# xmindflow/cenet

Hardware: AMD Instinct MI355X
Metric: training images/sec (224x224, 4-class) (higher is better)
Workload: dtype bf16

## Files before the change

cenet_amd/csrc/pvt_mlp.hip:

```cpp
#include "gemm_ring.h"

struct PvtMlpArgs {
  const bf16_t* x;
  const float* ln_g;
  const float* ln_b;
  const bf16_t* w1;
  const float* b1;
  const float* wd;
  const float* bd;
  const bf16_t* w2;
  const float* b2;
  const float* bscale;
  bf16_t* y;
  bf16_t* xn_out;
  float* mean_out;
  float* rstd_out;
  bf16_t* h_out;
  bf16_t* a_out;
  int H, W, HD, tiles_x, tiles_per_img;
  float eps;
};

#ifdef CENET_HOSTSIM_BUILD
#define PVT_WAVE_ID(tid) ((tid) >> 6)
#else
#define PVT_WAVE_ID(tid) __builtin_amdgcn_readfirstlane((tid) >> 6)
#endif

__device__ __forceinline__ float pvt_rcp(float x) {
#ifdef CENET_HOSTSIM_BUILD
  return 1.f / x;
#else
  return __builtin_amdgcn_rcpf(x);
#endif
}
__device__ __forceinline__ float pvt_gelu(float u) { return gelu_as(u); }
template <int LPT>
__device__ __forceinline__ float pvt_subrow_sum(float v) {
#pragma unroll
  for (int o = LPT / 2; o > 0; o >>= 1) v += __shfl_xor(v, o);
  return v;
}

__device__ __forceinline__ void pvt_load_kf64(const bf16_t* src, long ld, unsigned char* img, int wave, int lane) {
  const int S = wave * 64 + lane, row = S >> 3, c = (S & 7) ^ kf_key(row);
  ring_glds16(src + (long)row * ld + 8 * c, img + wave * 1024, lane);
}

template <int BX>
__device__ __forceinline__ void pvt_load_rf(const bf16_t* src, long ld, unsigned char* img, int wave, int lane) {
  constexpr int CH = BX / 8;
#pragma unroll
  for (int j = 0; j < BX / 64; ++j) {
    const int S = (j * 8 + wave) * 64 + lane;
    const int k = S / CH, c = (S % CH) ^ rf_key<BX>(k);
    ring_glds16(src + (long)k * ld + 8 * c, img + (j * 8 + wave) * 1024, lane);
  }
}

template <int C, int PW, int PT, int PTP, int TH, int TW>
__device__ __forceinline__ void pvt_ln_tile(const bf16_t* ximg, const float* ln_g, const float* ln_b, float eps, int H, int W,
                                            int y0, int x0, int halo, unsigned char* XN, bf16_t* xn_out, float* mean_out,
                                            float* rstd_out, int tid) {
  constexpr int LPT = C / 8, TPP = 512 / LPT;
  const int j = tid % LPT, tsub = tid / LPT;
  float gm[8], bt[8];
  {
    const f4 g0 = ld4(ln_g + 8 * j), g1 = ld4(ln_g + 8 * j + 4), b0 = ld4(ln_b + 8 * j), b1 = ld4(ln_b + 8 * j + 4);
#pragma unroll
    for (int e = 0; e < 4; ++e) gm[e] = g0.v[e], gm[4 + e] = g1.v[e], bt[e] = b0.v[e], bt[4 + e] = b1.v[e];
  }
  const float invC = 1.f / C;
#pragma unroll
  for (int p0 = 0; p0 < PTP; p0 += TPP) {
    const int p = p0 + tsub;
    const int ty = p / PW, tx = p - ty * PW;
    const int iy = y0 - halo + ty, ix = x0 - halo + tx;
    const bool ok = p < PT && iy >= 0 && iy < H && ix >= 0 && ix < W;
    float v[8];
    if (ok) ldv<8>(v, ximg + ((long)iy * W + ix) * C + 8 * j);
    else {
#pragma unroll
      for (int e = 0; e < 8; ++e) v[e] = 0.f;
    }
    float s = ((v[0] + v[1]) + (v[2] + v[3])) + ((v[4] + v[5]) + (v[6] + v[7]));
    const float mu = pvt_subrow_sum<LPT>(s) * invC;
    float q = 0.f;
#pragma unroll
    for (int e = 0; e < 8; ++e) {
      const float d = v[e] - mu;
      q += d * d;
    }
    const float rs = rsqrtf(pvt_subrow_sum<LPT>(q) * invC + eps);
    unsigned o[4];
#pragma unroll
    for (int h = 0; h < 4; ++h) {
      const float a0 = ok ? (v[2 * h] - mu) * rs * gm[2 * h] + bt[2 * h] : 0.f;
      const float a1 = ok ? (v[2 * h + 1] - mu) * rs * gm[2 * h + 1] + bt[2 * h + 1] : 0.f;
      o[h] = cenet_pack_bf2(a0, a1);
    }
    if (p < PTP) *(uint4*)(XN + (j >> 3) * (PTP * 128) + p * 128 + ((j & 7) ^ kf_key(p)) * 16) = uint4{o[0], o[1], o[2], o[3]};
    if (xn_out && ok && ty >= halo && ty < halo + TH && tx >= halo && tx < halo + TW) {
      const long tk = (long)iy * W + ix;
      *(uint4*)(xn_out + tk * C + 8 * j) = uint4{o[0], o[1], o[2], o[3]};
      if (j == 0) mean_out[tk] = mu, rstd_out[tk] = rs;
    }
  }
}

template <int C, int TH, int TW>
struct PvtFwdGeo {
  static constexpr int PW = TW + 2, PH = TH + 2, PT = PH * PW, PTP = (PT + 15) / 16 * 16, MTH = PTP / 16;
  static constexpr int NT = TH * TW, MTI = (NT + 15) / 16, SL = TW / 2;
  static constexpr int KB = C / 64, HS = 136;
  static constexpr int XN_B = KB * PTP * 128, A_B = MTI * 16 * 128, W1_B = KB * 8192, W2_B = C * 128, H_B = PTP * HS;
  static constexpr int O_XN = 0, O_A = XN_B, O_W1 = O_A + A_B, O_W2 = O_W1 + W1_B, O_H = O_W2 + W2_B, LDS = O_H + H_B;
};

template <int C, int TH, int TW>
__global__ __launch_bounds__(512, 2) void pvt_mlp_fwd_kernel(PvtMlpArgs a) {
  typedef PvtFwdGeo<C, TH, TW> G;
  constexpr int PW = G::PW, PT = G::PT, PTP = G::PTP, MTH = G::MTH, NT = G::NT, MTI = G::MTI, SL = G::SL, KB = G::KB, HS = G::HS;
  static_assert(C == 64 || C == 128, "channels");
  static_assert(MTI <= 8 && 2 * TH <= 16 && TW % 2 == 0, "tile shape");
  __shared__ __attribute__((aligned(1024))) unsigned char lds[G::LDS];
  unsigned char* const XN = lds + G::O_XN;
  unsigned char* const AI = lds + G::O_A;
  unsigned char* const W1I = lds + G::O_W1;
  unsigned char* const W2I = lds + G::O_W2;
  unsigned char* const HI = lds + G::O_H;

  const int tid = threadIdx.x, lane = tid & 63;
  const int wave = PVT_WAVE_ID(tid);
  const cenet_bid bid = cenet_xcd_block();
  const int b = bid.x / a.tiles_per_img, t = bid.x - b * a.tiles_per_img;
  const int y0 = (t / a.tiles_x) * TH, x0 = (t % a.tiles_x) * TW;
  const long img = (long)b * a.H * a.W;
  const bf16_t* ximg = a.x + img * C;
  const int nslab = a.HD / 64;

#pragma unroll
  for (int kb = 0; kb < KB; ++kb) pvt_load_kf64(a.w1 + kb * 64, C, W1I + kb * 8192, wave, lane);
#pragma unroll
  for (int r = 0; r < C / 64; ++r) pvt_load_kf64(a.w2 + (long)(r * 64) * a.HD, a.HD, W2I + r * 8192, wave, lane);

  pvt_ln_tile<C, PW, PT, PTP, TH, TW>(ximg, a.ln_g, a.ln_b, a.eps, a.H, a.W, y0, x0, 1, XN, a.xn_out ? a.xn_out + img * C : nullptr,
                                      a.mean_out + img, a.rstd_out + img, tid);

  f32x4 acc[C / 16];
#pragma unroll
  for (int i = 0; i < C / 16; ++i) acc[i] = f32x4{0.f, 0.f, 0.f, 0.f};

  const float sc_b = a.bscale ? a.bscale[b] : 1.f;
  const int cp = tid & 31, strip = tid >> 5;
  const int oy = strip >> 1, ox0 = (strip & 1) * SL;
  const bool p2_on = strip < 2 * TH;
  const int ct = wave & 3;

  ring_wait_vm<0>();
  __syncthreads();

  for (int s = 0; s < nslab; ++s) {
    float wdv[18], bdv[2], b1v[4];
    {
      const float* wp = a.wd + (long)(s * 64 + 2 * cp) * 9;
#pragma unroll
      for (int i = 0; i < 9; ++i) {
        const float2 v = *(const float2*)(wp + 2 * i);
        wdv[2 * i] = v.x, wdv[2 * i + 1] = v.y;
      }
      bdv[0] = a.bd[s * 64 + 2 * cp], bdv[1] = a.bd[s * 64 + 2 * cp + 1];
      const f4 bb = ld4(a.b1 + s * 64 + ct * 16 + (lane >> 4) * 4);
      b1v[0] = bb.v[0], b1v[1] = bb.v[1], b1v[2] = bb.v[2], b1v[3] = bb.v[3];
    }
    {
      bf16x8 wf[KB * 2];
#pragma unroll
      for (int k = 0; k < KB * 2; ++k) wf[k] = ring_frag_kf(W1I + (k >> 1) * 8192, ct * 16, k & 1, lane);
      for (int tt = wave >> 2; tt < MTH; tt += 2) {
        f32x4 h = f32x4{0.f, 0.f, 0.f, 0.f};
#pragma unroll
        for (int k = 0; k < KB * 2; ++k) {
          const bf16x8 xf = ring_frag_kf(XN + (k >> 1) * (PTP * 128), tt * 16, k & 1, lane);
          h = __builtin_amdgcn_mfma_f32_16x16x32_bf16(wf[k], xf, h, 0, 0, 0);
        }
        const int p = tt * 16 + (lane & 15);
        const int ty = p / PW, tx = p - ty * PW;
        const int iy = y0 - 1 + ty, ix = x0 - 1 + tx;
        const bool ok = p < PT && iy >= 0 && iy < a.H && ix >= 0 && ix < a.W;
        unsigned o[2];
        o[0] = ok ? cenet_pack_bf2(h[0] + b1v[0], h[1] + b1v[1]) : 0u;
        o[1] = ok ? cenet_pack_bf2(h[2] + b1v[2], h[3] + b1v[3]) : 0u;
        *(uint2*)(HI + p * HS + (ct * 16 + (lane >> 4) * 4) * 2) = uint2{o[0], o[1]};
      }
    }
    __syncthreads();
    if (s + 1 < nslab) {
#pragma unroll
      for (int kb = 0; kb < KB; ++kb) pvt_load_kf64(a.w1 + (long)(s + 1) * 64 * C + kb * 64, C, W1I + kb * 8192, wave, lane);
    }
    unsigned hkeep[SL], akeep[SL];
    if (p2_on) {
      float u[SL][2];
#pragma unroll
      for (int i = 0; i < SL; ++i) u[i][0] = bdv[0], u[i][1] = bdv[1];
      const unsigned char* hp = HI + (oy * PW + ox0) * HS + cp * 4;
#pragma unroll
      for (int kxx = 0; kxx < SL + 2; ++kxx) {
        float h0[3], h1[3];
#pragma unroll
        for (int ky = 0; ky < 3; ++ky) {
          const unsigned v = *(const unsigned*)(hp + (ky * PW + kxx) * HS);
          h0[ky] = __uint_as_float(v << 16);
          h1[ky] = __uint_as_float(v & 0xFFFF0000u);
          if (ky == 1 && kxx >= 1 && kxx <= SL) hkeep[kxx - 1] = v;
        }
#pragma unroll
        for (int kx = 0; kx < 3; ++kx) {
          const int i = kxx - kx;
          if (i >= 0 && i < SL) {
#pragma unroll
            for (int ky = 0; ky < 3; ++ky) {
              u[i][0] += wdv[ky * 3 + kx] * h0[ky];
              u[i][1] += wdv[9 + ky * 3 + kx] * h1[ky];
            }
          }
        }
      }
#pragma unroll
      for (int i = 0; i < SL; ++i) {
        const int row = oy * TW + ox0 + i;
        const float a0 = pvt_gelu(u[i][0]), a1 = pvt_gelu(u[i][1]);
        const unsigned v = cenet_pack_bf2(a0, a1);
        *(unsigned*)(AI + row * 128 + (((cp >> 2) ^ kf_key(row)) * 16) + (cp & 3) * 4) = v;
        akeep[i] = a.bscale ? cenet_pack_bf2(a0 * sc_b, a1 * sc_b) : v;
      }
    }
    ring_wait_vm<0>();
    __syncthreads();
    if (a.h_out && p2_on) {
      const long o = (img + (long)(y0 + oy) * a.W + x0 + ox0) * a.HD + s * 64 + 2 * cp;
#pragma unroll
      for (int i = 0; i < SL; ++i) {
        *(unsigned*)(a.h_out + o + (long)i * a.HD) = hkeep[i];
        *(unsigned*)(a.a_out + o + (long)i * a.HD) = akeep[i];
      }
    }
    if (wave < MTI) {
#pragma unroll
      for (int kc = 0; kc < 2; ++kc) {
        const bf16x8 af = ring_frag_kf(AI, wave * 16, kc, lane);
#pragma unroll
        for (int nt = 0; nt < C / 16; ++nt) {
          const bf16x8 wf = ring_frag_kf(W2I + (nt >> 2) * 8192, (nt & 3) * 16, kc, lane);
          acc[nt] = __builtin_amdgcn_mfma_f32_16x16x32_bf16(wf, af, acc[nt], 0, 0, 0);
        }
      }
    }
    __syncthreads();
    if (s + 1 < nslab) {
#pragma unroll
      for (int r = 0; r < C / 64; ++r)
        pvt_load_kf64(a.w2 + (long)(r * 64) * a.HD + (s + 1) * 64, a.HD, W2I + r * 8192, wave, lane);
    }
  }
  if (wave < MTI) {
    const int ti = wave * 16 + (lane & 15);
    const int ry = ti / TW, rx = ti - ry * TW;
    const int gy = y0 + ry, gx = x0 + rx;
    if (ti < NT && gy < a.H && gx < a.W) {
      const float sc = sc_b;
      const long tok = img + (long)gy * a.W + gx;
#pragma unroll
      for (int nt = 0; nt < C / 16; ++nt) {
        const int n0 = nt * 16 + (lane >> 4) * 4;
        const f4 xr = ld4(a.x + tok * C + n0);
        const f4 bb = ld4(a.b2 + n0);
        f4 o;
#pragma unroll
        for (int e = 0; e < 4; ++e) o.v[e] = xr.v[e] + sc * (acc[nt][e] + bb.v[e]);
        st4(a.y + tok * C + n0, o);
      }
    }
  }
}

__device__ __forceinline__ float pvt_gelu_grad(float u) { return gelu_as_grad(u); }

struct PvtBwdArgs {
  const bf16_t* g;
  const float* bscale;
  const bf16_t* w1;
  const bf16_t* w2;
  const float* wd;
  const float* bd;
  const bf16_t* h;
  bf16_t* gu;
  bf16_t* dh;
  float* dwd;
  float* dbd;
  const bf16_t* x;
  const float* ln_g;
  const float* mean;
  const float* rstd;
  bf16_t* dx;
  const float* up_scale;
  bf16_t* dxs;
  float* ws;
  int H, W, HD, tiles_x, tiles_per_img, tpw;
};

template <int ROWS, typename F>
__device__ __forceinline__ void pvt_dma_plane(const bf16_t* base, long ld, unsigned char* plane, int wave, int lane, F tok) {
  constexpr int NI = (ROWS * 8 + 511) / 512;
#pragma unroll
  for (int j = 0; j < NI; ++j) {
    const int S = (j * 8 + wave) * 64 + lane, p = S >> 3, c = S & 7;
    if ((j * 8 + wave) * 64 < ROWS * 8) {
      const long t = p < ROWS ? tok(p) : -1;
      ring_glds16(t >= 0 ? (const void*)(base + t * ld + 8 * c) : (const void*)ring_zero16, plane + (j * 8 + wave) * 1024, lane);
    }
  }
}

template <int C, int TH, int TW>
struct PvtB1Geo {
  static constexpr int PW = TW + 2, PH = TH + 2, PT = PH * PW, NT = TH * TW, MTI = (NT + 15) / 16, SL = TW / 2;
  static constexpr int KB = C / 64, KS = C / 32, HS = 136;
  static constexpr int HP_B = (PT * 128 + 1023) / 1024 * 1024, GS_B = KB * MTI * 16 * 128, W2_B = KB * 8192, DA_B = MTI * 16 * HS;
  static constexpr int O_HP = 0, O_GS = 2 * HP_B, O_W2 = O_GS + GS_B, O_DA = O_W2 + W2_B, LDS = O_DA + DA_B;
};

template <int C, int TH, int TW>
__global__ __launch_bounds__(512, 4) void pvt_mlp_bwd1_kernel(PvtBwdArgs a) {
  typedef PvtB1Geo<C, TH, TW> G;
  constexpr int PW = G::PW, PT = G::PT, NT = G::NT, MTI = G::MTI, SL = G::SL, KB = G::KB, KS = G::KS, HS = G::HS;
  static_assert(G::LDS >= 8 * 32 * 20 * 4, "the end-of-kernel reduction reuses the buffers");
  __shared__ __attribute__((aligned(1024))) unsigned char lds[G::LDS];
  unsigned char* const GS = lds + G::O_GS;
  unsigned char* const W2R = lds + G::O_W2;
  unsigned char* const DA = lds + G::O_DA;
  const int tid = threadIdx.x, lane = tid & 63;
  const int wave = PVT_WAVE_ID(tid);
  const cenet_bid bid = cenet_xcd_block();
  const int s = bid.x, b = bid.z;
  const long img = (long)b * a.H * a.W;
  const float sc = a.bscale ? a.bscale[b] : 1.f;
  const int cp = tid & 31, strip = tid >> 5;
  const int oy = strip >> 1, ox0 = (strip & 1) * SL;
  const bool on = strip < 2 * TH;
  const int ct = wave & 3;

#pragma unroll
  for (int kb = 0; kb < KB; ++kb) pvt_load_rf<64>(a.w2 + (long)(kb * 64) * a.HD + s * 64, a.HD, W2R + kb * 8192, wave, lane);
  float wdv[18], wacc[2][10];
  {
    const float* wp = a.wd + (long)(s * 64 + 2 * cp) * 9;
#pragma unroll
    for (int i = 0; i < 9; ++i) {
      const float2 v = *(const float2*)(wp + 2 * i);
      wdv[2 * i] = v.x, wdv[2 * i + 1] = v.y;
    }
#pragma unroll
    for (int e = 0; e < 2; ++e)
#pragma unroll
      for (int k = 0; k < 10; ++k) wacc[e][k] = 0.f;
  }
  const float bd0 = a.bd[s * 64 + 2 * cp], bd1 = a.bd[s * 64 + 2 * cp + 1];

  const int t_begin = bid.y * a.tpw;
  const int t_end = t_begin + a.tpw < a.tiles_per_img ? t_begin + a.tpw : a.tiles_per_img;
  auto issue_h = [&](int tile, int buf) __attribute__((always_inline)) {
    const int y0 = (tile / a.tiles_x) * TH, x0 = (tile % a.tiles_x) * TW;
    pvt_dma_plane<PT>(a.h + img * a.HD + s * 64, a.HD, lds + G::O_HP + buf * G::HP_B, wave, lane, [&](int p) -> long {
      const int ty = p / PW, tx = p - ty * PW;
      const int iy = y0 - 1 + ty, ix = x0 - 1 + tx;
      return (iy >= 0 && iy < a.H && ix >= 0 && ix < a.W) ? (long)iy * a.W + ix : -1;
    });
  };
  auto issue_g = [&](int tile) __attribute__((always_inline)) {
    const int y0 = (tile / a.tiles_x) * TH, x0 = (tile % a.tiles_x) * TW;
    constexpr int NI = (MTI * 16 * 8 + 511) / 512;
#pragma unroll
    for (int kb = 0; kb < KB; ++kb)
#pragma unroll
      for (int j = 0; j < NI; ++j) {
        if ((j * 8 + wave) * 64 < MTI * 16 * 8) {
          const int S = (j * 8 + wave) * 64 + lane, ti = S >> 3, c = (S & 7) ^ kf_key(ti);
          const int ry = ti / TW, rx = ti - ry * TW;
          const bool ok = ti < NT && y0 + ry < a.H && x0 + rx < a.W;
          const void* src = ok ? (const void*)(a.g + (img + (long)(y0 + ry) * a.W + x0 + rx) * C + kb * 64 + 8 * c)
                               : (const void*)ring_zero16;
          ring_glds16(src, GS + kb * (MTI * 16 * 128) + (j * 8 + wave) * 1024, lane);
        }
      }
  };
  issue_h(t_begin, 0);
  issue_g(t_begin);
  int buf = 0;
  for (int tile = t_begin; tile < t_end; ++tile, buf ^= 1) {
    const int y0 = (tile / a.tiles_x) * TH, x0 = (tile % a.tiles_x) * TW;
    ring_wait_vm<0>();
    __syncthreads();
    if (tile + 1 < t_end) issue_h(tile + 1, buf ^ 1);
    for (int tt = wave >> 2; tt < MTI; tt += 2) {
      f32x4 d = f32x4{0.f, 0.f, 0.f, 0.f};
#pragma unroll
      for (int k = 0; k < KS; ++k) {
        const bf16x8 wf = ring_frag_rf<64>(W2R + (k >> 1) * 8192, ct * 16, k & 1, lane);
        const bf16x8 gf = ring_frag_kf(GS + (k >> 1) * (MTI * 16 * 128), tt * 16, k & 1, lane);
        d = __builtin_amdgcn_mfma_f32_16x16x32_bf16(wf, gf, d, 0, 0, 0);
      }
      const int p = tt * 16 + (lane & 15);
      *(uint2*)(DA + p * HS + (ct * 16 + (lane >> 4) * 4) * 2) =
          uint2{cenet_pack_bf2(sc * d[0], sc * d[1]), cenet_pack_bf2(sc * d[2], sc * d[3])};
    }
    __syncthreads();
    if (tile + 1 < t_end) issue_g(tile + 1);
    if (on) {
      const unsigned char* hp = lds + G::O_HP + buf * G::HP_B + (oy * PW + ox0) * 128 + cp * 4;
      float win[3][3][2];
#pragma unroll
      for (int kxx = 0; kxx < 2; ++kxx)
#pragma unroll
        for (int ky = 0; ky < 3; ++ky) {
          const unsigned v = *(const unsigned*)(hp + (ky * PW + kxx) * 128);
          win[ky][kxx][0] = __uint_as_float(v << 16);
          win[ky][kxx][1] = __uint_as_float(v & 0xFFFF0000u);
        }
      bf16_t* const gup = a.gu + (img + (long)(y0 + oy) * a.W + x0 + ox0) * a.HD + s * 64 + 2 * cp;
#pragma unroll
      for (int i = 0; i < SL; ++i) {
#pragma unroll
        for (int ky = 0; ky < 3; ++ky) {
          const unsigned v = *(const unsigned*)(hp + (ky * PW + i + 2) * 128);
          win[ky][2][0] = __uint_as_float(v << 16);
          win[ky][2][1] = __uint_as_float(v & 0xFFFF0000u);
        }
        float u0 = bd0, u1 = bd1;
#pragma unroll
        for (int ky = 0; ky < 3; ++ky)
#pragma unroll
          for (int kx = 0; kx < 3; ++kx) {
            u0 += wdv[ky * 3 + kx] * win[ky][kx][0];
            u1 += wdv[9 + ky * 3 + kx] * win[ky][kx][1];
          }
        const int row = oy * TW + ox0 + i;
        const unsigned dv = *(const unsigned*)(DA + row * HS + cp * 4);
        const float g0 = __uint_as_float(dv << 16) * pvt_gelu_grad(u0);
        const float g1 = __uint_as_float(dv & 0xFFFF0000u) * pvt_gelu_grad(u1);
        *(unsigned*)(gup + (long)i * a.HD) = cenet_pack_bf2(g0, g1);
#pragma unroll
        for (int ky = 0; ky < 3; ++ky)
#pragma unroll
          for (int kx = 0; kx < 3; ++kx) {
            wacc[0][ky * 3 + kx] += g0 * win[ky][kx][0];
            wacc[1][ky * 3 + kx] += g1 * win[ky][kx][1];
          }
        wacc[0][9] += g0;
        wacc[1][9] += g1;
#pragma unroll
        for (int ky = 0; ky < 3; ++ky) {
          win[ky][0][0] = win[ky][1][0], win[ky][0][1] = win[ky][1][1];
          win[ky][1][0] = win[ky][2][0], win[ky][1][1] = win[ky][2][1];
        }
      }
    }
    __syncthreads();
  }
  float* red = (float*)lds;
#pragma unroll
  for (int e = 0; e < 2; ++e)
#pragma unroll
    for (int k = 0; k < 10; ++k) wacc[e][k] += __shfl_xor(wacc[e][k], 32);
  if (lane < 32) {
#pragma unroll
    for (int e = 0; e < 2; ++e)
#pragma unroll
      for (int k = 0; k < 10; ++k) red[(wave * 32 + cp) * 20 + e * 10 + k] = wacc[e][k];
  }
  __syncthreads();
  for (int i = tid; i < 640; i += 512) {
    const int ch = i / 10, k = i - ch * 10;
    float v = 0.f;
#pragma unroll
    for (int w = 0; w < 8; ++w) v += red[(w * 32 + (ch >> 1)) * 20 + (ch & 1) * 10 + k];
    if (k < 9) atomicAdd(&a.dwd[(long)(s * 64 + ch) * 9 + k], v);
    else atomicAdd(&a.dbd[s * 64 + ch], v);
  }
}

template <int C, int TH, int TW>
struct PvtB2Geo {
  static constexpr int PW = TW + 2, PH = TH + 2, PT = PH * PW, NT = TH * TW, MTI = (NT + 15) / 16, SL = TW / 2;
  static constexpr int GU_B = (PT * 128 + 1023) / 1024 * 1024, W1_B = 64 * C * 2, DH_B = MTI * 16 * 128;
  static constexpr int O_GU = 0, O_W1 = 2 * GU_B, O_DH = O_W1 + 2 * W1_B, O_LN = O_DH + DH_B, LDS = O_LN + 3 * C * 4;
};

template <int C, int TH, int TW>
__global__ __launch_bounds__(512, C == 64 ? 4 : 2) void pvt_mlp_bwd2_kernel(PvtBwdArgs a) {
  typedef PvtB2Geo<C, TH, TW> G;
  constexpr int PW = G::PW, PT = G::PT, NT = G::NT, MTI = G::MTI, SL = G::SL;
  __shared__ __attribute__((aligned(1024))) unsigned char lds[G::LDS];
  unsigned char* const DH = lds + G::O_DH;
  float* const LNS = (float*)(lds + G::O_LN);
  const int tid = threadIdx.x, lane = tid & 63;
  const int wave = PVT_WAVE_ID(tid);
  const cenet_bid bid = cenet_xcd_block();
  const int b = bid.x / a.tiles_per_img, t = bid.x - b * a.tiles_per_img;
  const int y0 = (t / a.tiles_x) * TH, x0 = (t % a.tiles_x) * TW;
  const long img = (long)b * a.H * a.W;
  const int nslab = a.HD / 64;
  const int cp = tid & 31, strip = tid >> 5;
  const int oy = strip >> 1, ox0 = (strip & 1) * SL;
  const bool on = strip < 2 * TH;
  for (int i = tid; i < 3 * C; i += 512) LNS[i] = 0.f;
  const float sc = a.bscale ? a.bscale[b] : 1.f;

  auto issue = [&](int s, int buf) __attribute__((always_inline)) {
    pvt_dma_plane<PT>(a.gu + img * a.HD + s * 64, a.HD, lds + G::O_GU + buf * G::GU_B, wave, lane, [&](int p) -> long {
      const int ty = p / PW, tx = p - ty * PW;
      const int iy = y0 - 1 + ty, ix = x0 - 1 + tx;
      return (iy >= 0 && iy < a.H && ix >= 0 && ix < a.W) ? (long)iy * a.W + ix : -1;
    });
    pvt_load_rf<C>(a.w1 + (long)s * 64 * C, C, lds + G::O_W1 + buf * G::W1_B, wave, lane);
  };
  f32x4 acc[C / 16];
#pragma unroll
  for (int i = 0; i < C / 16; ++i) acc[i] = f32x4{0.f, 0.f, 0.f, 0.f};
  issue(0, 0);
  float wdv[18];
  {
    const float* wp = a.wd + (long)(2 * cp) * 9;
#pragma unroll
    for (int i = 0; i < 9; ++i) {
      const float2 v = *(const float2*)(wp + 2 * i);
      wdv[2 * i] = v.x, wdv[2 * i + 1] = v.y;
    }
  }
  for (int s = 0, buf = 0; s < nslab; ++s, buf ^= 1) {
    ring_wait_vm<0>();
    __syncthreads();
    if (s + 1 < nslab) issue(s + 1, buf ^ 1);
    float wdn[18];
    {
      const float* wp = a.wd + (long)((s + 1 < nslab ? s + 1 : s) * 64 + 2 * cp) * 9;
#pragma unroll
      for (int i = 0; i < 9; ++i) {
        const float2 v = *(const float2*)(wp + 2 * i);
        wdn[2 * i] = v.x, wdn[2 * i + 1] = v.y;
      }
    }
    if (on) {
      float dhv[SL][2];
#pragma unroll
      for (int i = 0; i < SL; ++i) dhv[i][0] = 0.f, dhv[i][1] = 0.f;
      const unsigned char* gp = lds + G::O_GU + buf * G::GU_B + (oy * PW + ox0) * 128 + cp * 4;
#pragma unroll
      for (int kxx = 0; kxx < SL + 2; ++kxx) {
        float d0[3], d1[3];
#pragma unroll
        for (int jy = 0; jy < 3; ++jy) {
          const unsigned v = *(const unsigned*)(gp + (jy * PW + kxx) * 128);
          d0[jy] = __uint_as_float(v << 16);
          d1[jy] = __uint_as_float(v & 0xFFFF0000u);
        }
#pragma unroll
        for (int jx = 0; jx < 3; ++jx) {
          const int i = kxx - jx;
          if (i >= 0 && i < SL) {
#pragma unroll
            for (int jy = 0; jy < 3; ++jy) {
              dhv[i][0] += wdv[(2 - jy) * 3 + (2 - jx)] * d0[jy];
              dhv[i][1] += wdv[9 + (2 - jy) * 3 + (2 - jx)] * d1[jy];
            }
          }
        }
      }
      bf16_t* const dhp = a.dh + (img + (long)(y0 + oy) * a.W + x0 + ox0) * a.HD + s * 64 + 2 * cp;
#pragma unroll
      for (int i = 0; i < SL; ++i) {
        const int row = oy * TW + ox0 + i;
        const unsigned v = cenet_pack_bf2(dhv[i][0], dhv[i][1]);
        *(unsigned*)(DH + row * 128 + (((cp >> 2) ^ kf_key(row)) * 16) + (cp & 3) * 4) = v;
        *(unsigned*)(dhp + (long)i * a.HD) = v;
      }
    }
#pragma unroll
    for (int i = 0; i < 18; ++i) wdv[i] = wdn[i];
    __syncthreads();
    if (wave < MTI) {
      const unsigned char* W1R = lds + G::O_W1 + buf * G::W1_B;
#pragma unroll
      for (int kc = 0; kc < 2; ++kc) {
        const bf16x8 hf = ring_frag_kf(DH, wave * 16, kc, lane);
#pragma unroll
        for (int nt = 0; nt < C / 16; ++nt) {
          const bf16x8 wf = ring_frag_rf<C>(W1R, nt * 16, kc, lane);
          acc[nt] = __builtin_amdgcn_mfma_f32_16x16x32_bf16(wf, hf, acc[nt], 0, 0, 0);
        }
      }
    }
  }
  if (wave < MTI) {
    const int ti = wave * 16 + (lane & 15);
    const int ry = ti / TW, rx = ti - ry * TW;
    const int gy = y0 + ry, gx = x0 + rx;
    const bool in = ti < NT && gy < a.H && gx < a.W;
    const long tok = img + (long)(in ? gy : y0) * a.W + (in ? gx : x0);
    const float mu = a.mean[tok], rs = a.rstd[tok];
    float xh[C / 16][4], qv[C / 16][4];
    float s1 = 0.f, s2 = 0.f;
#pragma unroll
    for (int nt = 0; nt < C / 16; ++nt) {
      const int n0 = nt * 16 + (lane >> 4) * 4;
      const f4 xr = ld4(a.x + tok * C + n0);
      const f4 gm = ld4(a.ln_g + n0);
#pragma unroll
      for (int e = 0; e < 4; ++e) {
        const float dxn = in ? acc[nt][e] : 0.f;
        xh[nt][e] = (xr.v[e] - mu) * rs;
        qv[nt][e] = dxn * gm.v[e];
        s1 += qv[nt][e];
        s2 += qv[nt][e] * xh[nt][e];
        float dg = dxn * xh[nt][e], db = dxn;
#pragma unroll
        for (int o = 8; o > 0; o >>= 1) dg += __shfl_xor(dg, o), db += __shfl_xor(db, o);
        if ((lane & 15) == 0) {
          atomicAdd(&LNS[n0 + e], dg);
          atomicAdd(&LNS[C + n0 + e], db);
        }
      }
    }
    s1 += __shfl_xor(s1, 16), s2 += __shfl_xor(s2, 16);
    s1 += __shfl_xor(s1, 32), s2 += __shfl_xor(s2, 32);
    const float m1 = s1 * (1.f / C), m2 = s2 * (1.f / C);
#pragma unroll
    for (int nt = 0; nt < C / 16; ++nt) {
      const int n0 = nt * 16 + (lane >> 4) * 4;
      const f4 gr = ld4(a.g + tok * C + n0);
      if (in) {
        f4 o;
#pragma unroll
        for (int e = 0; e < 4; ++e) o.v[e] = gr.v[e] + rs * (qv[nt][e] - m1 - xh[nt][e] * m2);
        st4(a.dx + tok * C + n0, o);
        if (a.dxs) {
          const float us = a.up_scale[b];
#pragma unroll
          for (int e = 0; e < 4; ++e) o.v[e] = us * cenet_bf2f(cenet_f2bf(o.v[e]));
          st4(a.dxs + tok * C + n0, o);
        }
      }
#pragma unroll
      for (int e = 0; e < 4; ++e) {
        float v = in ? sc * gr.v[e] : 0.f;
#pragma unroll
        for (int o = 8; o > 0; o >>= 1) v += __shfl_xor(v, o);
        if ((lane & 15) == 0) atomicAdd(&LNS[2 * C + n0 + e], v);
      }
    }
  }
  __syncthreads();
  for (int i = tid; i < 3 * C; i += 512) a.ws[(long)bid.x * 3 * C + i] = LNS[i];
}

__global__ __launch_bounds__(256) void pvt_mlp_lnfold_kernel(const float* __restrict__ ws, int rows, int C, float* __restrict__ dg,
                                                            float* __restrict__ db, float* __restrict__ db2) {
  __shared__ float red[256];
  const int c = blockIdx.x, tid = threadIdx.x;
  float s = 0.f;
  for (int r = tid; r < rows; r += 256) s += ws[(long)r * 3 * C + c];
  red[tid] = s;
  __syncthreads();
  for (int o = 128; o > 0; o >>= 1) {
    if (tid < o) red[tid] += red[tid + o];
    __syncthreads();
  }
  if (tid == 0) {
    if (c < C) dg[c] += red[0];
    else if (c < 2 * C) db[c - C] += red[0];
    else if (db2) db2[c - 2 * C] += red[0];
  }
}

struct PvtMlpPlan {
  int TH, TW, tiles_x, tiles_per_img;
  int k1th, k1_tiles_per_img, k1_tpw, k1_runs;
};
static bool pvt_mlp_geo(int H, int W, PvtMlpPlan& p) {
  if (H <= 0 || W <= 0 || W % 14 != 0) return false;
  p.TW = 14;
  if (H % 8 == 0) p.TH = 8;
  else if (H % 7 == 0) p.TH = 7;
  else return false;
  p.tiles_x = W / p.TW;
  p.tiles_per_img = p.tiles_x * (H / p.TH);
  return true;
}

extern "C" int cenet_pvt_mlp_supported(int C, int HD, int H, int W) {
  PvtMlpPlan p;
  return (C == 64 || C == 128) && HD % 64 == 0 && HD >= 64 && pvt_mlp_geo(H, W, p) ? 1 : 0;
}

static int pvt_mlp_plan(int B, int H, int W, int C, int HD, PvtMlpPlan& p) {
  if (B <= 0) return CENET_EINVAL;
  if (!cenet_pvt_mlp_supported(C, HD, H, W) || !pvt_mlp_geo(H, W, p)) return CENET_EUNSUPPORTED;
  p.k1th = p.TH == 7 && H % 4 == 0 ? 4 : p.TH;
  p.k1_tiles_per_img = p.tiles_x * (H / p.k1th);
  int runs = 1024 / ((HD / 64) * B);
  if (runs < 1) runs = 1;
  p.k1_tpw = cdiv(p.k1_tiles_per_img, runs);
  p.k1_runs = cdiv(p.k1_tiles_per_img, p.k1_tpw);
  return CENET_OK;
}

extern "C" int cenet_pvt_mlp_bwd_plan(int B, int H, int W, int C, int HD, int* tile_rows, int* k1_tile_rows,
                                      int* k1_tiles_per_run, int* k1_runs) {
  PvtMlpPlan p;
  const int rc = pvt_mlp_plan(B, H, W, C, HD, p);
  if (rc != CENET_OK) return rc;
  if (tile_rows) *tile_rows = p.TH;
  if (k1_tile_rows) *k1_tile_rows = p.k1th;
  if (k1_tiles_per_run) *k1_tiles_per_run = p.k1_tpw;
  if (k1_runs) *k1_runs = p.k1_runs;
  return CENET_OK;
}

extern "C" int cenet_pvt_mlp_fwd_bf16(const bf16_t* x, const float* ln_g, const float* ln_b, float eps, const bf16_t* w1,
                                      const float* b1, const float* wd, const float* bd, const bf16_t* w2, const float* b2,
                                      const float* bscale, bf16_t* y, bf16_t* xn_out, float* mean_out, float* rstd_out,
                                      bf16_t* h_out, bf16_t* a_out, int B, int H, int W, int C, int HD, hipStream_t stream) {
  if (!x || !ln_g || !ln_b || !w1 || !b1 || !wd || !bd || !w2 || !b2 || !y || B <= 0) return CENET_EINVAL;
  const int nsave = (xn_out != nullptr) + (mean_out != nullptr) + (rstd_out != nullptr) + (h_out != nullptr) + (a_out != nullptr);
  if (nsave != 0 && nsave != 5) return CENET_EINVAL;
  if ((((uintptr_t)xn_out | (uintptr_t)h_out | (uintptr_t)a_out) & 15) != 0) return CENET_EUNSUPPORTED;
  PvtMlpPlan pl;
  if (const int rc = pvt_mlp_plan(B, H, W, C, HD, pl)) return rc;
  const int TH = pl.TH;
  if ((((uintptr_t)x | (uintptr_t)y | (uintptr_t)w1 | (uintptr_t)w2 | (uintptr_t)ln_g | (uintptr_t)ln_b | (uintptr_t)b1 |
        (uintptr_t)b2) & 15) != 0 || (((uintptr_t)wd | (uintptr_t)bd) & 7) != 0)
    return CENET_EUNSUPPORTED;
  PvtMlpArgs a = {};
  a.x = x; a.ln_g = ln_g; a.ln_b = ln_b; a.w1 = w1; a.b1 = b1; a.wd = wd; a.bd = bd; a.w2 = w2; a.b2 = b2; a.bscale = bscale;
  a.y = y; a.xn_out = xn_out; a.mean_out = mean_out; a.rstd_out = rstd_out; a.h_out = h_out; a.a_out = a_out;
  a.H = H; a.W = W; a.HD = HD; a.eps = eps;
  a.tiles_x = pl.tiles_x;
  a.tiles_per_img = pl.tiles_per_img;
  const dim3 grid(B * a.tiles_per_img);
#define PVT_FWD_GO(C_, TH_)                                                                  \
  if (C == C_ && TH == TH_) {                                                                 \
    CENET_LAUNCH((pvt_mlp_fwd_kernel<C_, TH_, 14>), grid, dim3(512), stream, a);              \
    CENET_CHECK_LAUNCH();                                                                     \
    return CENET_OK;                                                                          \
  }
  PVT_FWD_GO(64, 8)
  PVT_FWD_GO(64, 7)
  PVT_FWD_GO(128, 8)
  PVT_FWD_GO(128, 7)
#undef PVT_FWD_GO
  return CENET_EUNSUPPORTED;
}


extern "C" long cenet_pvt_mlp_bwd_ws_floats(int B, int H, int W, int C) {
  PvtMlpPlan pl;
  if (!pvt_mlp_geo(H, W, pl)) return 0;
  return (long)B * pl.tiles_per_img * 3 * C;
}

extern "C" int cenet_pvt_mlp_bwd_bf16(const bf16_t* g, const float* bscale, const bf16_t* w1, const bf16_t* w2, const float* wd,
                                      const float* bd, const bf16_t* h, const bf16_t* x, const float* ln_g, const float* mean,
                                      const float* rstd, bf16_t* gu, bf16_t* dh, bf16_t* dx, const float* up_scale, bf16_t* dxs,
                                      float* dwd_acc, float* dbd_acc, float* dln_g_acc, float* dln_b_acc, float* db2_acc,
                                      float* ws, int B, int H, int W, int C, int HD, hipStream_t stream) {
  if (!g || !w1 || !w2 || !wd || !bd || !h || !x || !ln_g || !mean || !rstd || !gu || !dh || !dx || !dwd_acc || !dbd_acc ||
      !dln_g_acc || !dln_b_acc || B <= 0 || (up_scale != nullptr) != (dxs != nullptr))
    return CENET_EINVAL;
  PvtMlpPlan pl;
  if (const int rc = pvt_mlp_plan(B, H, W, C, HD, pl)) return rc;
  if (!ws) return CENET_EINVAL;
  const int TH = pl.TH, k1th = pl.k1th;
  if ((((uintptr_t)g | (uintptr_t)h | (uintptr_t)x | (uintptr_t)gu | (uintptr_t)dh | (uintptr_t)dx | (uintptr_t)dxs |
        (uintptr_t)w1 | (uintptr_t)w2 | (uintptr_t)ln_g) & 15) != 0 || (((uintptr_t)wd | (uintptr_t)bd) & 7) != 0)
    return CENET_EUNSUPPORTED;
  PvtBwdArgs a = {};
  a.g = g; a.bscale = bscale; a.w1 = w1; a.w2 = w2; a.wd = wd; a.bd = bd; a.h = h; a.gu = gu; a.dh = dh;
  a.dwd = dwd_acc; a.dbd = dbd_acc; a.x = x; a.ln_g = ln_g; a.mean = mean; a.rstd = rstd; a.dx = dx; a.ws = ws;
  a.up_scale = up_scale; a.dxs = dxs;
  a.H = H; a.W = W; a.HD = HD;
  a.tiles_x = pl.tiles_x;
  a.tiles_per_img = pl.tiles_per_img;
  PvtBwdArgs a1 = a;
  a1.tiles_per_img = pl.k1_tiles_per_img;
  a1.tpw = pl.k1_tpw;
  const dim3 g1(HD / 64, pl.k1_runs, B), g2(B * a.tiles_per_img);
  if (g1.y > 65535 || g1.z > 65535) return CENET_EUNSUPPORTED;
#define PVT_BWD_GO(C_, TH_)                                                                              \
  if (C == C_ && TH == TH_) {                                                                             \
    if (k1th == 4) CENET_LAUNCH((pvt_mlp_bwd1_kernel<C_, 4, 14>), g1, dim3(512), stream, a1);             \
    else CENET_LAUNCH((pvt_mlp_bwd1_kernel<C_, TH_, 14>), g1, dim3(512), stream, a1);                     \
    CENET_LAUNCH((pvt_mlp_bwd2_kernel<C_, TH_, 14>), g2, dim3(512), stream, a);                           \
  } else
  PVT_BWD_GO(64, 8)
  PVT_BWD_GO(64, 7)
  PVT_BWD_GO(128, 8)
  PVT_BWD_GO(128, 7)
  return CENET_EUNSUPPORTED;
#undef PVT_BWD_GO
  CENET_LAUNCH(pvt_mlp_lnfold_kernel, dim3(3 * C), dim3(256), stream, (const float*)ws, (int)g2.x, C, dln_g_acc, dln_b_acc, db2_acc);
  CENET_CHECK_LAUNCH();
  return CENET_OK;
}
```

Measured before the change: 1930.

## Batch LDS transpose reads, use lighter barriers, and drop per-tile trailing sync in PVT MLP backward

Rewrites the MFMA fragment loads in both PVT MLP backward kernels to use precomputed-address ds_read_b64_tr_b16 with immediate offsets. All fragments are issued before the MFMAs, so LDS latency is batched. Full __syncthreads are replaced with lgkmcnt-only waits plus s_barrier, the trailing per-tile barrier in bwd1 is removed, and occupancy launch bounds now depend on LDS size. The depthwise weight prefetch moves later, and scheduling fences are added in the stencil loop. Removing the trailing barrier and relaxing the waits both risk LDS hazards between tiles, and batching fragments raises register pressure.

```diff
diff --git a/cenet_amd/csrc/pvt_mlp.hip b/cenet_amd/csrc/pvt_mlp.hip
--- a/cenet_amd/csrc/pvt_mlp.hip
+++ b/cenet_amd/csrc/pvt_mlp.hip
@@ -310,6 +310,77 @@
   int H, W, HD, tiles_x, tiles_per_img, tpw;
 };
 
+template <int I>
+struct pvt_ic {
+  static constexpr int value = I;
+};
+template <int N, typename F>
+__device__ __forceinline__ void pvt_static_for(F f) {
+  if constexpr (N > 0) {
+    pvt_static_for<N - 1>(f);
+    f(pvt_ic<N - 1>{});
+  }
+}
+
+template <int BX>
+__device__ __forceinline__ unsigned pvt_rf_addr(const unsigned char* img, int r0, int lane) {
+#ifdef CENET_HOSTSIM_BUILD
+  (void)img, (void)r0, (void)lane;
+  return 0;
+#else
+  static_assert(BX == 64 || BX == 128, "row-fast image width");
+  constexpr int CH = BX / 8;
+  const int g = lane >> 4, i = lane & 15, q = i >> 2, p = i & 3;
+  const int x = r0 + 4 * p, k = 8 * g + q;
+  const unsigned char* a = img + (k * CH + ((x >> 3) ^ rf_key<BX>(k))) * 16 + (x & 7) * 2;
+  return (unsigned)(__UINTPTR_TYPE__)(const __attribute__((address_space(3))) unsigned char*)a;
+#endif
+}
+template <int BX, int IMG, int KC>
+__device__ __forceinline__ bf16x8 pvt_frag_rf(const unsigned char* img, int r0, int lane, unsigned a0) {
+#ifdef CENET_HOSTSIM_BUILD
+  (void)a0;
+  return ring_frag_rf<BX>(img + IMG, r0, KC, lane);
+#else
+  (void)img, (void)r0, (void)lane;
+  constexpr int CH = BX / 8;
+  static_assert(IMG + (KC * 32 + 4) * CH * 16 < 65536, "offset field");
+  bf16x8 f;
+  ring_s4 v0, v1;
+  asm volatile("ds_read_b64_tr_b16 %0, %1 offset:%2" : "=v"(v0) : "v"(a0), "n"(IMG + KC * 32 * CH * 16));
+  asm volatile("ds_read_b64_tr_b16 %0, %1 offset:%2" : "=v"(v1) : "v"(a0), "n"(IMG + (KC * 32 + 4) * CH * 16));
+  f[0] = v0[0], f[1] = v0[1], f[2] = v0[2], f[3] = v0[3];
+  f[4] = v1[0], f[5] = v1[1], f[6] = v1[2], f[7] = v1[3];
+  return f;
+#endif
+}
+__device__ __forceinline__ void pvt_lds_store(unsigned char* p, unsigned v) {
+#ifdef CENET_HOSTSIM_BUILD
+  *(unsigned*)p = v;
+#else
+  asm volatile("ds_write_b32 %0, %1" ::"v"((unsigned)(__UINTPTR_TYPE__)(__attribute__((address_space(3))) unsigned char*)p), "v"(v) : "memory");
+#endif
+}
+__device__ __forceinline__ void pvt_lds_store(unsigned char* p, uint2 v) {
+#ifdef CENET_HOSTSIM_BUILD
+  *(uint2*)p = v;
+#else
+  asm volatile("ds_write_b64 %0, %1" ::"v"((unsigned)(__UINTPTR_TYPE__)(__attribute__((address_space(3))) unsigned char*)p), "v"(v) : "memory");
+#endif
+}
+__device__ __forceinline__ void pvt_phase_barrier() {
+#ifdef CENET_HOSTSIM_BUILD
+  __syncthreads();
+#else
+  asm volatile("s_waitcnt lgkmcnt(0)\n\ts_barrier" ::: "memory");
+#endif
+}
+__device__ __forceinline__ void pvt_step_fence() {
+#ifndef CENET_HOSTSIM_BUILD
+  __builtin_amdgcn_sched_barrier(0);
+#endif
+}
+
 template <int ROWS, typename F>
 __device__ __forceinline__ void pvt_dma_plane(const bf16_t* base, long ld, unsigned char* plane, int wave, int lane, F tok) {
   constexpr int NI = (ROWS * 8 + 511) / 512;
@@ -329,10 +400,11 @@
   static constexpr int KB = C / 64, KS = C / 32, HS = 136;
   static constexpr int HP_B = (PT * 128 + 1023) / 1024 * 1024, GS_B = KB * MTI * 16 * 128, W2_B = KB * 8192, DA_B = MTI * 16 * HS;
   static constexpr int O_HP = 0, O_GS = 2 * HP_B, O_W2 = O_GS + GS_B, O_DA = O_W2 + W2_B, LDS = O_DA + DA_B;
+  static constexpr int WPS = 2 * LDS <= 160 * 1024 ? 4 : 2;
 };
 
 template <int C, int TH, int TW>
-__global__ __launch_bounds__(512, 4) void pvt_mlp_bwd1_kernel(PvtBwdArgs a) {
+__global__ __launch_bounds__(512, (PvtB1Geo<C, TH, TW>::WPS)) void pvt_mlp_bwd1_kernel(PvtBwdArgs a) {
   typedef PvtB1Geo<C, TH, TW> G;
   constexpr int PW = G::PW, PT = G::PT, NT = G::NT, MTI = G::MTI, SL = G::SL, KB = G::KB, KS = G::KS, HS = G::HS;
   static_assert(G::LDS >= 8 * 32 * 20 * 4, "the end-of-kernel reduction reuses the buffers");
@@ -397,6 +469,7 @@
   };
   issue_h(t_begin, 0);
   issue_g(t_begin);
+  const unsigned w2a = pvt_rf_addr<64>(W2R, ct * 16, lane);
   int buf = 0;
   for (int tile = t_begin; tile < t_end; ++tile, buf ^= 1) {
     const int y0 = (tile / a.tiles_x) * TH, x0 = (tile % a.tiles_x) * TW;
@@ -405,17 +478,21 @@
     if (tile + 1 < t_end) issue_h(tile + 1, buf ^ 1);
     for (int tt = wave >> 2; tt < MTI; tt += 2) {
       f32x4 d = f32x4{0.f, 0.f, 0.f, 0.f};
-#pragma unroll
-      for (int k = 0; k < KS; ++k) {
-        const bf16x8 wf = ring_frag_rf<64>(W2R + (k >> 1) * 8192, ct * 16, k & 1, lane);
-        const bf16x8 gf = ring_frag_kf(GS + (k >> 1) * (MTI * 16 * 128), tt * 16, k & 1, lane);
-        d = __builtin_amdgcn_mfma_f32_16x16x32_bf16(wf, gf, d, 0, 0, 0);
-      }
+      bf16x8 wf[KS], gf[KS];
+      pvt_static_for<KS>([&](auto K) __attribute__((always_inline)) {
+        constexpr int k = decltype(K)::value;
+        wf[k] = pvt_frag_rf<64, (k >> 1) * 8192, k & 1>(W2R, ct * 16, lane, w2a);
+        gf[k] = ring_frag_kf(GS + (k >> 1) * (MTI * 16 * 128), tt * 16, k & 1, lane);
+      });
+#pragma unroll
+      for (int k = 0; k < KS; ++k) ring_frag_landed<false>(wf[k]);
+#pragma unroll
+      for (int k = 0; k < KS; ++k) d = __builtin_amdgcn_mfma_f32_16x16x32_bf16(wf[k], gf[k], d, 0, 0, 0);
       const int p = tt * 16 + (lane & 15);
-      *(uint2*)(DA + p * HS + (ct * 16 + (lane >> 4) * 4) * 2) =
-          uint2{cenet_pack_bf2(sc * d[0], sc * d[1]), cenet_pack_bf2(sc * d[2], sc * d[3])};
-    }
-    __syncthreads();
+      pvt_lds_store(DA + p * HS + (ct * 16 + (lane >> 4) * 4) * 2,
+                    uint2{cenet_pack_bf2(sc * d[0], sc * d[1]), cenet_pack_bf2(sc * d[2], sc * d[3])});
+    }
+    pvt_phase_barrier();
     if (tile + 1 < t_end) issue_g(tile + 1);
     if (on) {
       const unsigned char* hp = lds + G::O_HP + buf * G::HP_B + (oy * PW + ox0) * 128 + cp * 4;
@@ -431,6 +508,7 @@
       bf16_t* const gup = a.gu + (img + (long)(y0 + oy) * a.W + x0 + ox0) * a.HD + s * 64 + 2 * cp;
 #pragma unroll
       for (int i = 0; i < SL; ++i) {
+        pvt_step_fence();
 #pragma unroll
         for (int ky = 0; ky < 3; ++ky) {
           const unsigned v = *(const unsigned*)(hp + (ky * PW + i + 2) * 128);
@@ -466,8 +544,8 @@
         }
       }
     }
-    __syncthreads();
-  }
+  }
+  __syncthreads();
   float* red = (float*)lds;
 #pragma unroll
   for (int e = 0; e < 2; ++e)
@@ -542,15 +620,6 @@
     ring_wait_vm<0>();
     __syncthreads();
     if (s + 1 < nslab) issue(s + 1, buf ^ 1);
-    float wdn[18];
-    {
-      const float* wp = a.wd + (long)((s + 1 < nslab ? s + 1 : s) * 64 + 2 * cp) * 9;
-#pragma unroll
-      for (int i = 0; i < 9; ++i) {
-        const float2 v = *(const float2*)(wp + 2 * i);
-        wdn[2 * i] = v.x, wdn[2 * i + 1] = v.y;
-      }
-    }
     if (on) {
       float dhv[SL][2];
 #pragma unroll
@@ -582,24 +651,32 @@
       for (int i = 0; i < SL; ++i) {
         const int row = oy * TW + ox0 + i;
         const unsigned v = cenet_pack_bf2(dhv[i][0], dhv[i][1]);
-        *(unsigned*)(DH + row * 128 + (((cp >> 2) ^ kf_key(row)) * 16) + (cp & 3) * 4) = v;
+        pvt_lds_store(DH + row * 128 + (((cp >> 2) ^ kf_key(row)) * 16) + (cp & 3) * 4, v);
         *(unsigned*)(dhp + (long)i * a.HD) = v;
       }
     }
-#pragma unroll
-    for (int i = 0; i < 18; ++i) wdv[i] = wdn[i];
-    __syncthreads();
+    {
+      const float* wp = a.wd + (long)((s + 1 < nslab ? s + 1 : s) * 64 + 2 * cp) * 9;
+#pragma unroll
+      for (int i = 0; i < 9; ++i) {
+        const float2 v = *(const float2*)(wp + 2 * i);
+        wdv[2 * i] = v.x, wdv[2 * i + 1] = v.y;
+      }
+    }
+    pvt_phase_barrier();
     if (wave < MTI) {
       const unsigned char* W1R = lds + G::O_W1 + buf * G::W1_B;
-#pragma unroll
-      for (int kc = 0; kc < 2; ++kc) {
+      pvt_static_for<2>([&](auto KC) __attribute__((always_inline)) {
+        constexpr int kc = decltype(KC)::value;
         const bf16x8 hf = ring_frag_kf(DH, wave * 16, kc, lane);
-#pragma unroll
-        for (int nt = 0; nt < C / 16; ++nt) {
-          const bf16x8 wf = ring_frag_rf<C>(W1R, nt * 16, kc, lane);
-          acc[nt] = __builtin_amdgcn_mfma_f32_16x16x32_bf16(wf, hf, acc[nt], 0, 0, 0);
-        }
-      }
+        bf16x8 wf[C / 16];
+#pragma unroll
+        for (int nt = 0; nt < C / 16; ++nt) wf[nt] = pvt_frag_rf<C, 0, kc>(W1R, nt * 16, lane, pvt_rf_addr<C>(W1R, nt * 16, lane));
+#pragma unroll
+        for (int nt = 0; nt < C / 16; ++nt) ring_frag_landed<false>(wf[nt]);
+#pragma unroll
+        for (int nt = 0; nt < C / 16; ++nt) acc[nt] = __builtin_amdgcn_mfma_f32_16x16x32_bf16(wf[nt], hf, acc[nt], 0, 0, 0);
+      });
     }
   }
   if (wave < MTI) {
```

Result: no change. 1937 (median of 6 runs) (+0.4%).
